# submarine0418/underwater_image_enhancement

Measured on AMD Instinct MI355X. Metric: megapixels/sec enhanced, higher is better.
Workload: dtype f32/f64

## Files before the change

underwater_image_enhancement_amd/csrc/common.h:

```cpp
#pragma once
#include <hip/hip_runtime.h>
#include <stddef.h>
#include <stdint.h>

#include "../../include/uwie.h"

namespace uwie {

void set_error(const char *fmt, ...);
#define UWIE_HIP_CHECK(expr)                                                            \
    do {                                                                                \
        hipError_t _e = (expr);                                                         \
        if (_e != hipSuccess) {                                                         \
            ::uwie::set_error("%s failed: %s (%s:%d)", #expr, hipGetErrorString(_e), __FILE__, __LINE__); \
            return UWIE_E_HIP;                                                          \
        }                                                                               \
    } while (0)
#define UWIE_LAUNCH_CHECK() UWIE_HIP_CHECK(hipGetLastError())
#define UWIE_REQUIRE(cond, msg)                 \
    do {                                        \
        if (!(cond)) {                          \
            ::uwie::set_error("%s", msg);       \
            return UWIE_E_INVALID;              \
        }                                       \
    } while (0)

constexpr int kCastBinadeMin = -2;
constexpr int kCastBinades = 34;

struct LabTables {
    uint16_t gamma[256];
    uint16_t cbrt[3072];
    int32_t fwd[9];
    uint8_t invgamma[4096];
    int32_t ltoyf[512];
    int32_t abtoxz[36864];
    int32_t inv[9];
};

struct CastTables {
    uint32_t R[kCastBinades][256];
    uint8_t tie[kCastBinades][256];
    uint32_t RT[256][kCastBinades];
    uint2 RT2[128][kCastBinades];
    uint8_t tiebin[256];
};

void build_lab_tables(LabTables *t);
void build_cast_tables(CastTables *t);

struct Profiler;
Profiler *prof_create();
void prof_destroy(Profiler *p);
void prof_enable(Profiler *p, bool on);
void prof_filter(Profiler *p, const char *name);
void prof_bind(Profiler *p);
int prof_collect(Profiler *p);
int prof_row(Profiler *p, int i, const char **name, double *ms, int *calls);
class ProfScope {
public:
    ProfScope(const char *name, hipStream_t st);
    ~ProfScope();
    ProfScope(const ProfScope &) = delete;

private:
    int rec_;
    hipStream_t st_;
};
#define UWIE_PROF_CAT2(a, b) a##b
#define UWIE_PROF_CAT(a, b) UWIE_PROF_CAT2(a, b)
#define UWIE_PROF(name, st) ::uwie::ProfScope UWIE_PROF_CAT(_uwie_prof_, __LINE__)(name, st)
#define UWIE_LAUNCH(kernel, grid, block, lds, st, ...)                      \
    do {                                                                    \
        UWIE_PROF(#kernel, st);                                             \
        hipLaunchKernelGGL(kernel, grid, block, lds, st, __VA_ARGS__);      \
    } while (0)

}

namespace uwie {
struct Tuning {
    int gf_pipe = 1;
    int gf_split = 1;
    int gf_bands = 0;
    int select_generic = 0;
    int restore_store = 0;
    int lin_predict3 = 0;
    int lin_cap = 0;
    int lin_no_predict = 0;
    int q_hist = 1;
    int lin_predict_shift = 0;
    int streams = 1;
    int canny_prepass = 1;
    int gf_fuse = 0;
    int rank_sweep = 1;
    int canny_fault_inject = 0;
    int exact_fused = 1;
    int entry_fuse = 1;
};
const Tuning &tune();
uwie_ctx *current_ctx();
}

struct uwie_ctx {
    int device;
    uwie::Tuning tune;
    bool attr_q_tail = false;
    bool attr_cast_resolve = false;
    int attr_gf_fast = 0;
    int attr_gf_split8 = 0;
    uwie::LabTables *d_lab;
    uwie::CastTables *d_cast;
    uwie::Profiler *prof;
    uint32_t *d_status = nullptr;
    hipStream_t aux[4];
    hipEvent_t fork, join[4];
    bool aux_ready;
};

namespace uwie {

struct Carver {
    char *base;
    size_t off;
    explicit Carver(void *b) : base(static_cast<char *>(b)), off(0) {}
    template <typename T>
    T *take(size_t count)
    {
        off = (off + 255) & ~size_t(255);
        T *p = base ? reinterpret_cast<T *>(base + off) : nullptr;
        off += count * sizeof(T);
        return p;
    }
    size_t total() const { return (off + 255) & ~size_t(255); }
};

static inline int cdiv(long long a, long long b) { return (int)((a + b - 1) / b); }
static inline int grid_for(size_t n, size_t cap = 8192)
{
    size_t g = (n + 255) / 256;
    if (g > cap) g = cap;
    return g < 1 ? 1 : (int)g;
}

struct Region {
    int32_t img, y0, x0, rows, cols;
};

struct Shape {
    int B, H, W;
    size_t npx() const { return (size_t)H * W; }
};

size_t cast_ws_bytes(Shape s);
struct EntryFuse {
    uint32_t *qpart;
    uint8_t *gray;
    int32_t *guess;
    int gray_shift;
};
int launch_cast_classify(uwie_ctx *ctx, const uint8_t *d_in, Shape s, int32_t *d_kind, float *d_mean, void *ws,
                         hipStream_t st, const EntryFuse *ef = nullptr);
size_t quad_part_bytes(Shape s);
int launch_quad_hist_reduce(const uint32_t *qpart, Shape s, uint32_t *d_hist, hipStream_t st);
int launch_set_kind(int32_t *d_kind, int B, int kind, hipStream_t st);
int launch_normalise_correct(const uint8_t *d_in, const int32_t *d_kind, float *d_out, Shape s, hipStream_t st);
int launch_quant_gray(const uint8_t *d_in, const int32_t *d_kind, uint8_t *d_gray, Shape s, int gray_shift,
                      hipStream_t st);

size_t airlight_ws_bytes(Shape s);
int launch_airlight(uwie_ctx *ctx, const uint8_t *d_in, const int32_t *d_kind, uint8_t *d_gray, Shape s, int min_size,
                    float *d_A, void *d_trace, void *ws, hipStream_t st, int make_gray_shift = 0, const uint32_t *qpart = nullptr);
bool entry_fuse_takes(Shape s, int min_size);

size_t canny_ws_bytes(Shape s);
int launch_canny(const uint8_t *d_gray, Shape s, const Region *d_regions, int nreg, int max_rows, int max_cols, int low,
                 int high, uint32_t *d_count, uint8_t *d_edges, void *ws, hipStream_t st, bool count_is_zeroed = false,
                 bool strong_is_zeroed = false, bool prepass_done = false);
bool gray_strong_takes(Shape s);
int launch_gray_strong(const uint8_t *d_in, const int32_t *d_kind, uint8_t *d_gray, Shape s, const Region *d_regions, int nreg,
                       int max_rows, int max_cols, int high, int gray_shift, void *ws, hipStream_t st);
int launch_hist_strong(const uint8_t *d_in, const uint8_t *d_gray, Shape s, const Region *d_regions, int nreg, int max_rows,
                       int max_cols, int high, uint32_t *d_hist, void *ws, hipStream_t st);
uint32_t *canny_strong_flags(void *ws, Shape s);
int launch_make_full_regions(Region *d_regions, Shape s, hipStream_t st);

int launch_region_stats(const uint8_t *d_in, const int32_t *d_kind, const Region *d_regs, int nreg, int max_rows,
                        int max_cols, Shape s, float *csum, int maxChunks, float *tot, float *mean, float *vtot,
                        hipStream_t st);
int launch_frame_hist(const uint8_t *d_in, Shape s, uint32_t *d_hist, hipStream_t st);
size_t features_ws_bytes(Shape s);
int launch_features_u8(const uint8_t *d_in, Shape s, float *d_out, void *ws, hipStream_t st);

// ... 165 lines not shown
```

underwater_image_enhancement_amd/csrc/k_guided_pipe.hip:

```cpp
#include "common.h"
#include "devutil.h"
#include "guided_wave.h"

#include <algorithm>
#include <cmath>
#include <type_traits>
#include <utility>

namespace uwie {

namespace {

#define UWIE_TRY_RC(call)               \
    do {                                \
        const int _rc = (call);         \
        if (_rc != UWIE_OK) return _rc; \
    } while (0)

#ifndef UWIE_GF_MINBAND
#define UWIE_GF_MINBAND 32
#endif
constexpr int kPipeSlots = 128;
struct PipeGeom {
    int H, W, band;
// ... 463 lines not shown
        if constexpr (S == 0) {
            const double o0 = x0, o1 = x1;
            x0 = b0; x1 = b1;
            b0 = o0; b1 = o1;
        } else rest.template swap_at<S - 1>(b0, b1);
    }
    __device__ __forceinline__ void clear() { x0 = x1 = 0.0; rest.clear(); }
};
template <>
struct RegRing<0> {
    template <int S> __device__ __forceinline__ void swap_at(double &, double &) {}
    __device__ __forceinline__ void clear() {}
};

template <int N, bool G>
struct RawRing {
    uint32_t t0, t1, g;
    RawRing<N - 1, G> rest;
    template <int S>
    __device__ __forceinline__ void swap_at(uint32_t &a0, uint32_t &a1, uint32_t &gg)
    {
        if constexpr (S == 0) {
            const uint32_t o0 = t0, o1 = t1;
            t0 = a0; t1 = a1;
            a0 = o0; a1 = o1;
            if constexpr (G) {
                const uint32_t og = g;
                g = gg;
                gg = og;
            }
        } else rest.template swap_at<S - 1>(a0, a1, gg);
    }
    template <int S>
    __device__ __forceinline__ void set_at(uint32_t a0, uint32_t a1, uint32_t gg)
    {
        if constexpr (S == 0) {
            t0 = a0; t1 = a1;
            if constexpr (G) g = gg;
        } else rest.template set_at<S - 1>(a0, a1, gg);
    }
};
template <bool G>
struct RawRing<0, G> {
    template <int S> __device__ __forceinline__ void swap_at(uint32_t &, uint32_t &, uint32_t &) {}
    template <int S> __device__ __forceinline__ void set_at(uint32_t, uint32_t, uint32_t) {}
};

#ifndef SPLIT_QUAD
#define SPLIT_QUAD 1
#endif
#ifndef SPLIT_MUL24
#define SPLIT_MUL24 1
#endif
__device__ __forceinline__ double dpp_next(double v)
{
    const int lo = __builtin_amdgcn_update_dpp(0, __double2loint(v), 0x130, 0xf, 0xf, true);
    const int hi = __builtin_amdgcn_update_dpp(0, __double2hiint(v), 0x130, 0xf, 0xf, true);
    return __hiloint2double(hi, lo);
}
__device__ __forceinline__ uint32_t dpp_next(uint32_t v)
{
    return (uint32_t)__builtin_amdgcn_update_dpp(0, (int)v, 0x130, 0xf, 0xf, true);
}
__device__ __forceinline__ double2 q_add(double2 a, double2 b) { return make_double2(a.x + b.x, a.y + b.y); }
__device__ __forceinline__ double2 q_sub(double2 a, double2 b) { return make_double2(a.x - b.x, a.y - b.y); }
__device__ __forceinline__ double2 q_next(double2 v) { return make_double2(dpp_next(v.x), dpp_next(v.y)); }
__device__ __forceinline__ uint2 q_add(uint2 a, uint2 b) { return make_uint2(a.x + b.x, a.y + b.y); }
__device__ __forceinline__ uint2 q_sub(uint2 a, uint2 b) { return make_uint2(a.x - b.x, a.y - b.y); }
__device__ __forceinline__ uint2 q_next(uint2 v) { return make_uint2(dpp_next(v.x), dpp_next(v.y)); }

template <int K>
struct SplitCfg {
    static constexpr bool RAWREG = K <= 16;
    static constexpr int NB = K % 3 == 0 ? 3 : K > 16 ? 2 : K % 5 == 0 ? 5 : 2;
    static constexpr int AR = K > 16 ? 3 : 0;
    static constexpr bool STAGE_FIRST = AR > 0;
    static constexpr int pad_bytes = 16 * (PipeCfg<K>::M + 1) > 128 ? 16 * (PipeCfg<K>::M + 1) : 128;
    static constexpr int s2_bytes = STAGE_FIRST ? 2048 : 2048 + pad_bytes;
    static constexpr int ring_lds_bytes = (K - AR) * (PipeCfg<K>::NL + 1) * 16;
    static_assert(!STAGE_FIRST || ring_lds_bytes >= pad_bytes, "the look-ahead must stay inside the allocation");
    static constexpr int lds_bytes = ring_lds_bytes + PipeCfg<K>::s1_doubles * 8 + s2_bytes;
};

__device__ __forceinline__ uint32_t fuse_t0_bits(const float *tab, uint32_t r, uint32_t g, uint32_t b, float omega, int pre_clip)
{
    const float dark = fminf(fminf(tab[r], tab[256 + g]), tab[512 + b]);
    float t = __fsub_rn(1.0f, __fmul_rn(omega, dark));
    if (pre_clip) t = fminf(fmaxf(t, 0.1f), 1.0f);
    return __float_as_uint(t);
}

template <int K, bool EDGE, typename TOut, bool FUSE = false>
__device__ __forceinline__ void split_body(const uint8_t *__restrict__ gray, const float *__restrict__ t0, TOut *__restrict__ tout,
                                           const SplitGeom &g, const PipeConsts &cs, char *lds, int3 bid, int lane_in = -1,
                                           const float *tab = nullptr, float omega = 0.0f, int pre_clip = 0)
{
    using C = PipeCfg<K>;
    constexpr int a = C::a, Lb = C::Lb, NV = C::NV, RC = K, NL = C::NL, M = C::M, SW = C::SW;
    constexpr int NB = SplitCfg<K>::NB;
    static_assert(RC % NB == 0, "the ring period must be a multiple of the row buffers");
    constexpr bool RAWREG = SplitCfg<K>::RAWREG;
    constexpr int NLp = NL + 1, EB = 16;
    constexpr int AR = SplitCfg<K>::AR;
    constexpr int ring_bytes = SplitCfg<K>::ring_lds_bytes;
    constexpr uint32_t stage_base = SplitCfg<K>::STAGE_FIRST ? 0u : (uint32_t)ring_bytes;
    constexpr uint32_t ring_base = SplitCfg<K>::STAGE_FIRST ? 3072u + 2048u : 0u;
    constexpr double K2 = (double)(K * K);
    const int lane = lane_in >= 0 ? lane_in : (int)threadIdx.x;
    const int H = g.H, W = g.W;
    const int x_lo = bid.x * NV;
    const int y_lo = g.y0 + bid.y * g.band;
    const int r_lo = y_lo - a;
    const size_t img = (size_t)bid.z * H * W;
    const uint32_t npx = (uint32_t)H * (uint32_t)W;
    constexpr uint32_t kTB = FUSE ? 3u : 4u;
    const __amdgpu_buffer_rsrc_t rT = FUSE ? pipe_rsrc(reinterpret_cast<const uint8_t *>(t0) + img * 3, npx * 3u) : pipe_rsrc(t0 + img, npx * 4u),
                                 rG = pipe_rsrc(gray + img, npx), rO = pipe_rsrc(tout + img, npx * (uint32_t)sizeof(TOut));
    const uint32_t pitch_t = (uint32_t)W * kTB, pitch_g = (uint32_t)W, pitch_o = (uint32_t)W * (uint32_t)sizeof(TOut);

    const int xo0 = x_lo + 2 * lane;
    int craw[2], fix_addr[2];
    bool fix_need[2], fix_odd[2];
    uint32_t ofs_t[2], ofs_g[2], ofs_o[2], ofs_q[2];
#pragma unroll
    for (int j = 0; j < 2; ++j) {
        const int sl = 2 * lane + j;
        craw[j] = EDGE ? pipe_reflect(x_lo - 2 * a + sl, W) : x_lo - 2 * a + sl;
        ofs_t[j] = (uint32_t)craw[j] * kTB;
        ofs_g[j] = (uint32_t)craw[j];
        ofs_o[j] = EDGE ? (uint32_t)min(xo0 + j, W - 1) : (uint32_t)min(xo0, W - 2);
        ofs_q[j] = sl < NV && xo0 + j < W ? (uint32_t)(xo0 + j) * (uint32_t)sizeof(TOut) : kNoStore;
        const int c = x_lo - a + sl, cr = pipe_reflect(c, W);
        const int sp = min(max(cr - (x_lo - a), 0), kPipeSlots - 1);
        fix_need[j] = EDGE && cr != c;
        fix_addr[j] = (sp >> 1) << 2;
        fix_odd[j] = sp & 1;
    }

    const uint32_t a_ring = pipe_opaque(ring_base + (uint32_t)min(lane, NLp - 1) * (uint32_t)EB);

#ifndef SPLIT_RAW_G
#define SPLIT_RAW_G 1
#endif
    constexpr bool RAWG = SPLIT_RAW_G && RAWREG && K == 15 && !FUSE;
    struct In {
        uint32_t te[2];
        uint32_t ge[2], go[2];
        uint32_t gl[2];
        uint32_t tl[2];
    };
    auto byte_of = [](const uint32_t (&v)[2], int c) { return EDGE ? v[c] : (c == 0 ? (v[0] & 255u) : (v[0] >> 8)); };
    static_assert(!FUSE || RAWREG, "the fused transmission keeps its rows in the register ring (no leaving-row reload)");
    auto load_rows = [&](uint32_t oe_t, uint32_t oe_g, uint32_t ol_t, uint32_t ol_g, uint32_t oo_g, In &in) {
        if constexpr (!RAWREG) {
            if constexpr (!EDGE) {
                const u32x2 tl = __builtin_amdgcn_raw_buffer_load_b64(rT, ofs_t[0], ol_t, 0);
                in.tl[0] = tl.x; in.tl[1] = tl.y;
            } else {
                in.tl[0] = (uint32_t)__builtin_amdgcn_raw_buffer_load_b32(rT, ofs_t[0], ol_t, 0);
                in.tl[1] = (uint32_t)__builtin_amdgcn_raw_buffer_load_b32(rT, ofs_t[1], ol_t, 0);
            }
        }
        if constexpr (!RAWG) {
            if constexpr (!EDGE) in.gl[0] = (uint16_t)__builtin_amdgcn_raw_buffer_load_b16(rG, ofs_g[0], ol_g, 0);
            else {
                in.gl[0] = (uint8_t)__builtin_amdgcn_raw_buffer_load_b8(rG, ofs_g[0], ol_g, 0);
                in.gl[1] = (uint8_t)__builtin_amdgcn_raw_buffer_load_b8(rG, ofs_g[1], ol_g, 0);
            }
        }
        if constexpr (!EDGE) {
            if constexpr (FUSE) {
                in.te[0] = (uint32_t)__builtin_amdgcn_raw_buffer_load_b32(rT, ofs_t[0], oe_t, 0);
                in.te[1] = (uint16_t)__builtin_amdgcn_raw_buffer_load_b16(rT, ofs_t[0] + 4u, oe_t, 0);
            } else {
                const u32x2 te = __builtin_amdgcn_raw_buffer_load_b64(rT, ofs_t[0], oe_t, 0);
                in.te[0] = te.x; in.te[1] = te.y;
            }
            in.ge[0] = (uint16_t)__builtin_amdgcn_raw_buffer_load_b16(rG, ofs_g[0], oe_g, 0);
            in.go[0] = (uint16_t)__builtin_amdgcn_raw_buffer_load_b16(rG, ofs_o[0], oo_g, 0);
            in.ge[1] = in.go[1] = 0;
        } else {
#pragma unroll
            for (int j = 0; j < 2; ++j) {
                if constexpr (FUSE) {
                    const uint32_t r = (uint8_t)__builtin_amdgcn_raw_buffer_load_b8(rT, ofs_t[j], oe_t, 0);
                    const uint32_t gg = (uint8_t)__builtin_amdgcn_raw_buffer_load_b8(rT, ofs_t[j] + 1u, oe_t, 0);
                    const uint32_t bb = (uint8_t)__builtin_amdgcn_raw_buffer_load_b8(rT, ofs_t[j] + 2u, oe_t, 0);
                    in.te[j] = r | (gg << 8) | (bb << 16);
                } else {
                    in.te[j] = (uint32_t)__builtin_amdgcn_raw_buffer_load_b32(rT, ofs_t[j], oe_t, 0);
                }
                in.ge[j] = (uint8_t)__builtin_amdgcn_raw_buffer_load_b8(rG, ofs_g[j], oe_g, 0);
                in.go[j] = (uint8_t)__builtin_amdgcn_raw_buffer_load_b8(rG, ofs_o[j], oo_g, 0);
            }
        }
    };
    auto te_bits = [&](const In &in, uint32_t (&tb)[2]) {
        if constexpr (!FUSE) {
            tb[0] = in.te[0]; tb[1] = in.te[1];
        } else if constexpr (!EDGE) {
            const uint32_t w0 = in.te[0], w1 = in.te[1];
            tb[0] = fuse_t0_bits(tab, w0 & 255u, (w0 >> 8) & 255u, (w0 >> 16) & 255u, omega, pre_clip);
            tb[1] = fuse_t0_bits(tab, w0 >> 24, w1 & 255u, (w1 >> 8) & 255u, omega, pre_clip);
        } else {
#pragma unroll
            for (int j = 0; j < 2; ++j)
                tb[j] = fuse_t0_bits(tab, in.te[j] & 255u, (in.te[j] >> 8) & 255u, (in.te[j] >> 16) & 255u, omega, pre_clip);
        }
    };

    double V1p[2] = {0.0, 0.0}, V1gp[2] = {0.0, 0.0};
    uint32_t Sg[2] = {0, 0}, Sgg[2] = {0, 0};
    double V2a[2] = {0.0, 0.0}, V2b[2] = {0.0, 0.0};
    RawRing<RAWREG ? RC : 0, RAWG> raw;
    auto prologue_row = [&](auto j_tag) {
        constexpr int J = decltype(j_tag)::value;
        const uint32_t row = (uint32_t)pipe_reflect(r_lo - a + J, H);
        uint32_t tb[2], gq[2];
#pragma unroll
        for (int c = 0; c < 2; ++c) {
            gq[c] = (uint8_t)__builtin_amdgcn_raw_buffer_load_b8(rG, ofs_g[c], row * pitch_g, 0);
            if constexpr (FUSE) {
                const uint32_t r = (uint8_t)__builtin_amdgcn_raw_buffer_load_b8(rT, ofs_t[c], row * pitch_t, 0);
                const uint32_t gg = (uint8_t)__builtin_amdgcn_raw_buffer_load_b8(rT, ofs_t[c] + 1u, row * pitch_t, 0);
                const uint32_t bb = (uint8_t)__builtin_amdgcn_raw_buffer_load_b8(rT, ofs_t[c] + 2u, row * pitch_t, 0);
                tb[c] = fuse_t0_bits(tab, r, gg, bb, omega, pre_clip);
            } else {
                tb[c] = (uint32_t)__builtin_amdgcn_raw_buffer_load_b32(rT, ofs_t[c], row * pitch_t, 0);
            }
            const double p = (double)__uint_as_float(tb[c]);
            Sg[c] += gq[c];
            Sgg[c] += gq[c] * gq[c];
            V1p[c] += p;
            V1gp[c] += (double)gq[c] * p;
        }
        if constexpr (RAWREG) raw.template set_at<J>(tb[0], tb[1], gq[0] | (gq[1] << 8));
    };
    [&]<int... J>(std::integer_sequence<int, J...>) { (prologue_row(IC<J>{}), ...); }(std::make_integer_sequence<int, RC>{});
    RegRing<RC> rb;
    rb.clear();
#pragma unroll
    for (int s = 0; s < RC - AR; ++s) *reinterpret_cast<double2 *>(lds + a_ring + (uint32_t)(s * NLp * EB)) = make_double2(0.0, 0.0);
    RegRing<AR> ra;
    ra.clear();

    const uint32_t a16 = pipe_opaque(stage_base + (uint32_t)lane * 16u);
    const uint32_t a8 = pipe_opaque(stage_base + 2048u + (uint32_t)lane * 8u);
    const double2 *pp1 = reinterpret_cast<const double2 *>(lds + a16), *vv1 = pp1 + SW;
    const uint2 *pi = reinterpret_cast<const uint2 *>(lds + a8), *vi = pi + SW;
    const double2 *pp2 = reinterpret_cast<const double2 *>(lds + a16 + 3072u), *vv2 = pp2 + SW;
    static_assert(C::s1_doubles * 8 == 3072 && (SplitCfg<K>::STAGE_FIRST || SplitCfg<K>::s2_bytes >= 2048 + 16 * (C::M + 1)), "staging layout");
    auto window2 = [&](const double2 *pp, const double2 *vv, double2 P, double2 v1, double2 (&o)[2]) {
        double2 m0 = pp[1], m1 = pp[2];
#pragma unroll
        for (int d = 3; d < M; d += 2) { const double2 t = pp[d]; m0.x += t.x; m0.y += t.y; }
#pragma unroll
        for (int d = 4; d < M; d += 2) { const double2 t = pp[d]; m1.x += t.x; m1.y += t.y; }
        const double2 f0 = vv[M];
        const double midx = m0.x + m1.x, midy = m0.y + m1.y;
        if constexpr (K & 1) {
            const double2 pm = pp[M];
            o[0] = make_double2((P.x + midx) + f0.x, (P.y + midy) + f0.y);
            o[1] = make_double2((v1.x + midx) + pm.x, (v1.y + midy) + pm.y);
        } else {
            o[0] = make_double2(P.x + midx, P.y + midy);
            o[1] = make_double2((v1.x + midx) + f0.x, (v1.y + midy) + f0.y);
        }
    };
    constexpr bool QUAD = SPLIT_QUAD != 0 && ((K & 1) || !(M & 1));
    static_assert(!QUAD || !(K & 1) || (M & 1), "odd windows: an odd number of pair sums on either side of the lane's own");
    double2 keep1 = make_double2(0.0, 0.0), keep2 = keep1;
    uint2 keepI = make_uint2(0u, 0u);
    auto stage_q = [&](auto *line, auto s0, auto s1, auto &keep) {
        const auto P = q_add(s0, s1);
        const auto Pn = q_next(P);
        const auto R = q_add(P, Pn);
        line[0] = R;
        if constexpr (K & 1) {
            line[SW] = s1;
            keep = q_add(s1, Pn);
        } else {
            line[SW] = s0;
            keep = R;
        }
    };
    auto window_q = [&](const auto *rr, auto keep, auto s0, auto s1, auto *o) {
        using T = decltype(keep);
        const T w = rr[SW + M];
        if constexpr (K & 1) {
            T mid = rr[2];
#pragma unroll
            for (int d = 4; d <= M - 3; d += 2) mid = q_add(mid, rr[d]);
            o[1] = q_add(q_add(keep, mid), rr[M - 1]);
            o[0] = q_add(q_sub(o[1], w), s0);
        } else if constexpr (!(M & 1)) {
            T mid = rr[2];
#pragma unroll
            for (int d = 4; d <= M - 2; d += 2) mid = q_add(mid, rr[d]);
            o[0] = q_add(keep, mid);
            o[1] = q_add(q_sub(o[0], s0), w);
        } else {
            T mid = rr[1];
#pragma unroll
            for (int d = 3; d <= M - 2; d += 2) mid = q_add(mid, rr[d]);
            o[0] = q_add(q_add(s0, s1), mid);
            o[1] = q_add(q_add(s1, mid), w);
        }
    };
    auto stage_v1 = [&]() {
        if constexpr (QUAD) {
            stage_q(const_cast<double2 *>(pp1), make_double2(V1p[0], V1gp[0]), make_double2(V1p[1], V1gp[1]), keep1);
            stage_q(const_cast<uint2 *>(pi), make_uint2(Sg[0], Sgg[0]), make_uint2(Sg[1], Sgg[1]), keepI);
        } else {
            const_cast<double2 *>(pp1)[0] = make_double2(V1p[0] + V1p[1], V1gp[0] + V1gp[1]);
            const_cast<double2 *>(vv1)[0] = make_double2(V1p[0], V1gp[0]);
            const_cast<uint2 *>(pi)[0] = make_uint2(Sg[0] + Sg[1], Sgg[0] + Sgg[1]);
            const_cast<uint2 *>(vi)[0] = make_uint2(Sg[0], Sgg[0]);
        }
    };

    auto step = [&](auto warm_tag, auto slot_tag, const In &in, uint32_t orow, bool row_ok) {
        constexpr bool WARM = decltype(warm_tag)::value;
        constexpr int S = decltype(slot_tag)::value;
        char *ring_p = lds + a_ring + (uint32_t)((S >= AR ? S - AR : 0) * NLp * EB);
        double2 oab[2] = {make_double2(0.0, 0.0), make_double2(0.0, 0.0)};
        if constexpr (!WARM) {
            if constexpr (QUAD) window_q(pp2, keep2, make_double2(V2a[0], V2b[0]), make_double2(V2a[1], V2b[1]), oab);
            else window2(pp2, vv2, make_double2(V2a[0] + V2a[1], V2b[0] + V2b[1]), make_double2(V2a[1], V2b[1]), oab);
        }
        double2 opg[2];
        if constexpr (QUAD) window_q(pp1, keep1, make_double2(V1p[0], V1gp[0]), make_double2(V1p[1], V1gp[1]), opg);
        else window2(pp1, vv1, make_double2(V1p[0] + V1p[1], V1gp[0] + V1gp[1]), make_double2(V1p[1], V1gp[1]), opg);
        uint32_t oG[2], oGG[2];
        if constexpr (QUAD) {
            uint2 oi[2];
            window_q(pi, keepI, make_uint2(Sg[0], Sgg[0]), make_uint2(Sg[1], Sgg[1]), oi);
            oG[0] = oi[0].x; oGG[0] = oi[0].y;
            oG[1] = oi[1].x; oGG[1] = oi[1].y;
        } else {
            const uint2 *ps = pi;
            uint2 m0 = ps[1], m1 = ps[2];
#pragma unroll
            for (int d = 3; d < M; d += 2) { m0.x += ps[d].x; m0.y += ps[d].y; }
#pragma unroll
            for (int d = 4; d < M; d += 2) { m1.x += ps[d].x; m1.y += ps[d].y; }
            const uint32_t midg = m0.x + m1.x, midgg = m0.y + m1.y;
            const uint2 f0 = vi[M];
            if constexpr (K & 1) {
                const uint2 pm = ps[M];
                oG[0] = Sg[0] + Sg[1] + midg + f0.x;   oGG[0] = Sgg[0] + Sgg[1] + midgg + f0.y;
                oG[1] = Sg[1] + midg + pm.x;           oGG[1] = Sgg[1] + midgg + pm.y;
            } else {
                oG[0] = Sg[0] + Sg[1] + midg;          oGG[0] = Sgg[0] + Sgg[1] + midgg;
                oG[1] = Sg[1] + midg + f0.x;           oGG[1] = Sgg[1] + midgg + f0.y;
            }
        }
        double2 la = make_double2(0.0, 0.0);
        if constexpr (S >= AR) la = *reinterpret_cast<const double2 *>(ring_p);

        if constexpr (!WARM) {
#pragma unroll
            for (int c = 0; c < 2; ++c) {
                const double gd = (double)byte_of(in.go, c);
                const double q = fmin(fmax(fma(oab[c].x * cs.kaI, gd, fma(oab[c].y, cs.kb, cs.b0)), 0.1), 1.0);
                const uint32_t oq = row_ok ? ofs_q[c] : kNoStore;
                if constexpr (std::is_same<TOut, double>::value)
                    __builtin_amdgcn_raw_buffer_store_b64(__builtin_bit_cast(u32x2, q), rO, oq, orow, 0);
                else
                    __builtin_amdgcn_raw_buffer_store_b32(__float_as_uint((float)q), rO, oq, orow, 0);
            }
        }
        double av[2], bv[2];
#pragma unroll
        for (int c = 0; c < 2; ++c) {
            constexpr bool MUL24 = SPLIT_MUL24 && 255 * 255 * K * K < (1 << 24);
            const uint32_t nvar = MUL24 ? __umul24(oGG[c], (uint32_t)(K * K)) - __umul24(oG[c], oG[c])
                                        : oGG[c] * (uint32_t)(K * K) - oG[c] * oG[c];
            const double D = fma((double)nvar, 1.0 / 255.0, cs.Ek);
            const double gd = (double)oG[c];
            const double ncov = fma(K2, opg[c].y, -(gd * opg[c].x));
            av[c] = ncov * pipe_rcp(D);
            bv[c] = fma(av[c] * (-1.0 / 255.0), gd, opg[c].x) * (1.0 / K2);
        }
        if constexpr (EDGE) {
            double fa[2] = {av[0], av[1]}, fb[2] = {bv[0], bv[1]};
#pragma unroll
            for (int c = 0; c < 2; ++c) {
                auto bp = [&](double v) {
                    const int lo = __builtin_amdgcn_ds_bpermute(fix_addr[c], __double2loint(v));
                    const int hi = __builtin_amdgcn_ds_bpermute(fix_addr[c], __double2hiint(v));
                    return __hiloint2double(hi, lo);
                };
                const double a0 = bp(av[0]), a1 = bp(av[1]), b0 = bp(bv[0]), b1 = bp(bv[1]);
                if (fix_need[c]) {
                    fa[c] = fix_odd[c] ? a1 : a0;
                    fb[c] = fix_odd[c] ? b1 : b0;
                }
            }
            av[0] = fa[0]; av[1] = fa[1];
            bv[0] = fb[0]; bv[1] = fb[1];
        }
        double lb0 = bv[0], lb1 = bv[1];
        rb.template swap_at<S>(lb0, lb1);
        if constexpr (S < AR) {
            la = make_double2(av[0], av[1]);
            ra.template swap_at<S>(la.x, la.y);
        }
        V2a[0] += av[0] - la.x; V2a[1] += av[1] - la.y;
        V2b[0] += bv[0] - lb0;  V2b[1] += bv[1] - lb1;
        uint32_t tbe[2];
        te_bits(in, tbe);
        uint32_t lt[2] = {tbe[0], tbe[1]}, lg = EDGE ? (in.ge[0] | (in.ge[1] << 8)) : in.ge[0];
        if constexpr (RAWREG) raw.template swap_at<S>(lt[0], lt[1], lg);
        else { lt[0] = in.tl[0]; lt[1] = in.tl[1]; }
        if constexpr (!RAWG) lg = EDGE ? (in.gl[0] | (in.gl[1] << 8)) : in.gl[0];
#pragma unroll
        for (int c = 0; c < 2; ++c) {
            const double pe = (double)__uint_as_float(tbe[c]), pl = (double)__uint_as_float(lt[c]);
            const uint32_t ge = byte_of(in.ge, c), gl = c == 0 ? (lg & 255u) : (lg >> 8);
            Sg[c] += ge - gl;
            Sgg[c] += ge * ge - gl * gl;
            V1p[c] += pe - pl;
            V1gp[c] += (double)ge * pe - (double)gl * pl;
        }

        pipe_sync();
        stage_v1();
        if constexpr (QUAD) {
            stage_q(const_cast<double2 *>(pp2), make_double2(V2a[0], V2b[0]), make_double2(V2a[1], V2b[1]), keep2);
        } else {
            const_cast<double2 *>(pp2)[0] = make_double2(V2a[0] + V2a[1], V2b[0] + V2b[1]);
            const_cast<double2 *>(vv2)[0] = make_double2(V2a[0], V2b[0]);
        }
        if constexpr (S >= AR) *reinterpret_cast<double2 *>(ring_p) = make_double2(av[0], av[1]);
        pipe_sync();
    };

    pipe_sync();
    stage_v1();
    pipe_sync();
    const int i0 = r_lo + 1;
    int re = i0 + Lb;
    int gr = i0 - Lb - 2;
    int yo = y_lo;
    auto issue = [&](In &fill) {
        asm volatile("" : "+s"(re), "+s"(gr), "+s"(yo));
        const uint32_t er = (uint32_t)pipe_reflect(re, H), lr = (uint32_t)pipe_reflect(re - RC, H);
        const uint32_t og = (uint32_t)min(max(gr, 0), H - 1);
        load_rows(er * pitch_t, er * pitch_g, lr * pitch_t, lr * pitch_g, og * pitch_g, fill);
        ++re;
        ++gr;
    };
    In buf[NB];
    [&]<int... Q>(std::integer_sequence<int, Q...>) { (issue(buf[Q]), ...); }(std::make_integer_sequence<int, NB - 1>{});
    auto one = [&](auto warm_tag, auto slot_tag, In &fill, const In &use) {
        issue(fill);
        step(warm_tag, slot_tag, use, (uint32_t)yo * pitch_o, yo < H);
        if constexpr (!decltype(warm_tag)::value) ++yo;
        __builtin_amdgcn_sched_barrier(0);
    };
    auto period = [&](auto warm_tag) {
        auto at = [&](auto slot_tag) {
            constexpr int S = decltype(slot_tag)::value;
            one(warm_tag, slot_tag, buf[(S + NB - 1) % NB], buf[S % NB]);
        };
        [&]<int... Q>(std::integer_sequence<int, Q...>) { (at(IC<Q>{}), ...); }(std::make_integer_sequence<int, RC>{});
    };
    period(std::true_type{});
    const int nper = (((int)bid.y == g.nbands - 1 ? g.y_end - y_lo : g.band) + RC - 1) / RC;
    for (int p = 0; p < nper; ++p) period(std::false_type{});
}


template <int K, typename TOut>
__global__ void __launch_bounds__(64) __attribute__((amdgpu_waves_per_eu(2, 2)))
k_guided_split(const uint8_t *__restrict__ gray, const float *__restrict__ t0, TOut *__restrict__ tout, SplitGeom g, PipeConsts cs)
{
    extern __shared__ double2 lds_raw[];
    char *lds = reinterpret_cast<char *>(lds_raw);
    int3 bid = {(int)blockIdx.x, (int)blockIdx.y, (int)blockIdx.z};
    if (g.xcd_fold) {
        const uint32_t gx = gridDim.x, gy = gridDim.y, n = gx * gy * gridDim.z;
        const uint32_t lin = blockIdx.x + gx * (blockIdx.y + gy * blockIdx.z);
        const uint32_t xcd = lin & 7u, idx = lin >> 3, q = n >> 3, r = n & 7u;
        const uint32_t log = (xcd < r ? xcd * (q + 1) : r * (q + 1) + (xcd - r) * q) + idx;
        bid.x = (int)(log % gx);
        bid.y = (int)((log / gx) % gy);
        bid.z = (int)(log / (gx * gy));
    }
    const int x_lo = bid.x * PipeCfg<K>::NV;
    const bool edge = x_lo - 2 * PipeCfg<K>::a < 0 || x_lo - 2 * PipeCfg<K>::a + kPipeSlots > g.W;
    if (edge) split_body<K, true, TOut>(gray, t0, tout, g, cs, lds, bid);
    else split_body<K, false, TOut>(gray, t0, tout, g, cs, lds, bid);
}

struct FuseT0Args {
    const uint8_t *rgb;
    const int32_t *kind;
    const float *A;
    float omega, norm_eps;
    int pre_clip;
};

template <int K, typename TOut>
__global__ void __launch_bounds__(512) __attribute__((amdgpu_waves_per_eu(2, 2)))
k_guided_split8(const uint8_t *__restrict__ gray, FuseT0Args fz, TOut *__restrict__ tout, SplitGeom g, PipeConsts cs, int nstrips)
{
    extern __shared__ double2 lds_raw[];
    char *lds = reinterpret_cast<char *>(lds_raw);
    constexpr int per_wave = SplitCfg<K>::lds_bytes;
    float *tab = reinterpret_cast<float *>(lds + 8 * per_wave);
    const int wave = __builtin_amdgcn_readfirstlane((int)(threadIdx.x >> 6)), lane = threadIdx.x & 63;
    int grp = (int)blockIdx.x, b = (int)blockIdx.z;
    if (g.xcd_fold) {
        const uint32_t gx = gridDim.x, n = gx * gridDim.z, lin = blockIdx.x + gx * blockIdx.z;
        const uint32_t xcd = lin & 7u, idx = lin >> 3, q = n >> 3, r = n & 7u;
        const uint32_t log = (xcd < r ? xcd * (q + 1) : r * (q + 1) + (xcd - r) * q) + idx;
        grp = (int)(log % gx);
        b = (int)(log / gx);
    }
    {
        const int kd = fz.kind ? fz.kind[b] : 0;
        for (int i = threadIdx.x; i < 768; i += 512) {
            const int c = i >> 8;
            tab[i] = px_val(i & 255, px_atten(kd, c)) / (fz.A[b * 3 + c] + fz.norm_eps);
        }
    }
    __syncthreads();
    const int item = grp * 8 + wave;
    if (item >= nstrips * g.nbands) return;
    const int3 bid = {item % nstrips, item / nstrips, b};
    const int x_lo = bid.x * PipeCfg<K>::NV;
    const bool edge = x_lo - 2 * PipeCfg<K>::a < 0 || x_lo - 2 * PipeCfg<K>::a + kPipeSlots > g.W;
    const float *t0 = reinterpret_cast<const float *>(fz.rgb);
    if (edge) split_body<K, true, TOut, true>(gray, t0, tout, g, cs, lds + wave * per_wave, bid, lane, tab, fz.omega, fz.pre_clip);
    else split_body<K, false, TOut, true>(gray, t0, tout, g, cs, lds + wave * per_wave, bid, lane, tab, fz.omega, fz.pre_clip);
}

template <int K, typename TOut>
int launch_split8(const uint8_t *d_gray, const FuseT0Args &fz, Shape s, const PipeConsts &cs, TOut *d_t, int y0, int band, int nbands,
                  int y_end, hipStream_t st)
{
    using C = PipeCfg<K>;
    constexpr int lds = 8 * SplitCfg<K>::lds_bytes + 768 * 4;
    static_assert(lds <= 160 * 1024, "eight strips and the table have to fit one CU");
#ifndef UWIE_SPLIT8_FOLD
#define UWIE_SPLIT8_FOLD 1
#endif
    SplitGeom g{s.H, s.W, y0, band, y_end, UWIE_SPLIT8_FOLD, nbands};
    const int nstrips = cdiv(s.W, C::NV);
    uwie_ctx *ctx = current_ctx();
    const int bit = std::is_same<TOut, double>::value ? 1 : 2;
    if (ctx && !(ctx->attr_gf_split8 & bit)) {
        UWIE_HIP_CHECK(hipFuncSetAttribute(reinterpret_cast<const void *>(&k_guided_split8<K, TOut>),
                                           hipFuncAttributeMaxDynamicSharedMemorySize, lds));
        ctx->attr_gf_split8 |= bit;
    }
    {
        UWIE_PROF("k_guided_split8", st);
        hipLaunchKernelGGL((k_guided_split8<K, TOut>), dim3(cdiv((long long)nstrips * nbands, 8), 1, s.B), dim3(512), (size_t)lds, st, d_gray,
                           fz, d_t, g, cs, nstrips);
    }
    UWIE_LAUNCH_CHECK();
    return UWIE_OK;
}

template <int K, typename TOut>
int launch_split(const uint8_t *d_gray, const float *d_t0, Shape s, const PipeConsts &cs, TOut *d_t, int y0, int band, int nbands,
                 int y_end, hipStream_t st)
{
    using C = PipeCfg<K>;
    constexpr int lds = SplitCfg<K>::lds_bytes;
#ifndef UWIE_SPLIT_FOLD
#define UWIE_SPLIT_FOLD 1
#endif
    SplitGeom g{s.H, s.W, y0, band, y_end, UWIE_SPLIT_FOLD, nbands};
    const int nstrips = cdiv(s.W, C::NV);
    {
        UWIE_PROF("k_guided_split", st);
        hipLaunchKernelGGL((k_guided_split<K, TOut>), dim3(nstrips, nbands, s.B), dim3(64), (size_t)lds, st, d_gray, d_t0, d_t, g, cs);
    }
    UWIE_LAUNCH_CHECK();
    return UWIE_OK;
}

template <int K, bool FX, typename TOut>
int launch_pipe(const uint8_t *d_gray, const float *d_t0, Shape s, const PipeConsts &cs, TOut *d_t, hipStream_t st,
                const int *border = nullptr)
{
    using C = PipeCfg<K>;
    constexpr int lds = C::lds_bytes(FX);
    const int nstrips = cdiv(s.W, C::NV);
    const int resident = 256 * std::max(1, std::min(8, (160 * 1024) / lds));
    int nbands = 1;
    if (tune().gf_bands > 0) nbands = tune().gf_bands;
    else {
        const long strips = (long)nstrips * s.B;
        if (strips < 12L * resident) nbands = (int)cdiv((size_t)(12L * resident), (size_t)strips);
        const int cap = std::max(1, s.H / (16 * (K - 1)));
        nbands = std::min(nbands, std::max(cap, (int)cdiv((size_t)(3L * resident), (size_t)strips)));
    }
    nbands = std::max(1, std::min(nbands, s.H / std::max(UWIE_GF_MINBAND, 2 * K)));
    PipeGeom g{};
    g.H = s.H; g.W = s.W;
    g.band = cdiv(s.H, nbands);
    int gy = cdiv(s.H, g.band);
    if (border) {
        g.iy0 = border[0]; g.iy1 = border[1]; g.iband = border[2];
        gy = 2 + border[3];
        g.is0 = border[4]; g.is1 = border[5];
    }
    {
        UWIE_PROF("k_guided_pipe", st);
        hipLaunchKernelGGL((k_guided_pipe<K, FX, TOut>), dim3(nstrips, gy, s.B), dim3(64), (size_t)lds, st, d_gray, d_t0, d_t, g, cs);
    }
    UWIE_LAUNCH_CHECK();
    return UWIE_OK;
}

}

bool guided_split_plan(Shape s, int k, int *iy0, int *band, int *nb, int *rows)
{
    if (rows) *rows = 0;
    if ((k != 10 && k != 15 && k != 20) || (s.W & 1) || !tune().gf_split) return false;
    if (s.W < 2 * k || s.H < 4 * k || s.B > 65535 || s.npx() >= ((size_t)1 << 27)) return false;
    const int RC = k, a = k / 2, Lb = k - 1 - a, NV = kPipeSlots - 2 * (k - 1);
    const bool odd = k & 1;
    *iy0 = odd ? 0 : 2 * a;
    const int periods = odd ? cdiv(s.H, RC) : (s.H - 2 * a - 2 * Lb) / RC;
    if (periods < 4) return false;
    const long strips = (long)cdiv(s.W, NV) * s.B;
    const bool forced = tune().gf_bands > 0;
    int n;
    if (forced) n = tune().gf_bands;
    else {
        n = (int)cdiv((size_t)(8L * 2048), (size_t)strips);
        n = std::min(n, std::max(1, periods * RC / 180));
    }
    n = std::max(1, std::min(n, periods));
    if (odd) {
        const int per_band = cdiv(periods, n);
        *band = RC * per_band;
        *nb = cdiv(periods, per_band);
        if (rows) *rows = s.H;
    } else {
        const int per_band = periods / n;
        *band = RC * per_band;
        *nb = periods / per_band;
        if (rows) *rows = periods * RC;
    }
    return forced || strips * n >= 1024;
}

bool guided_fused_takes(Shape s, int k)
{
    if (k != 15 || !tune().gf_pipe || !tune().gf_fuse) return false;
    int iy0, band, nb, rows;
// ... 114 lines not shown
```

Measured before the change: 57010.

## Compute fused dark-channel transmission in registers and enable guided-filter fusion by default

The fused guided-filter split kernel now computes the initial transmission from RGB directly in registers, using per-image reciprocal divisors (StretchDiv) and packed float2 math. This replaces the per-block LDS lookup table that was built by 512-thread blocks. The kernel goes back to 64-thread single-strip blocks that use the normal split LDS footprint, and it computes the next row's transmission one step ahead to hide ALU latency. gf_fuse is switched on by default, so the fused path that skips a separate t0 pass now runs. In exchange there is more per-pixel arithmetic and register pressure, and a slower exact-division variant is used when the fast divisor is not valid.

Measured after the change: 59170, median of 6. 1.04x the previous value.

```diff
diff --git a/underwater_image_enhancement_amd/csrc/common.h b/underwater_image_enhancement_amd/csrc/common.h
--- a/underwater_image_enhancement_amd/csrc/common.h
+++ b/underwater_image_enhancement_amd/csrc/common.h
@@ -92,7 +92,7 @@
     int lin_predict_shift = 0;
     int streams = 1;
     int canny_prepass = 1;
-    int gf_fuse = 0;
+    int gf_fuse = 1;
     int rank_sweep = 1;
     int canny_fault_inject = 0;
     int exact_fused = 1;
@@ -108,7 +108,6 @@
     bool attr_q_tail = false;
     bool attr_cast_resolve = false;
     int attr_gf_fast = 0;
-    int attr_gf_split8 = 0;
     uwie::LabTables *d_lab;
     uwie::CastTables *d_cast;
     uwie::Profiler *prof;
diff --git a/underwater_image_enhancement_amd/csrc/k_guided_pipe.hip b/underwater_image_enhancement_amd/csrc/k_guided_pipe.hip
--- a/underwater_image_enhancement_amd/csrc/k_guided_pipe.hip
+++ b/underwater_image_enhancement_amd/csrc/k_guided_pipe.hip
@@ -569,18 +569,72 @@
     static constexpr int lds_bytes = ring_lds_bytes + PipeCfg<K>::s1_doubles * 8 + s2_bytes;
 };
 
-__device__ __forceinline__ uint32_t fuse_t0_bits(const float *tab, uint32_t r, uint32_t g, uint32_t b, float omega, int pre_clip)
-{
-    const float dark = fminf(fminf(tab[r], tab[256 + g]), tab[512 + b]);
-    float t = __fsub_rn(1.0f, __fmul_rn(omega, dark));
-    if (pre_clip) t = fminf(fmaxf(t, 0.1f), 1.0f);
-    return __float_as_uint(t);
-}
-
-template <int K, bool EDGE, typename TOut, bool FUSE = false>
+struct FuseT0Args {
+    const uint8_t *rgb;
+    const int32_t *kind;
+    const float *A;
+    float omega, norm_eps;
+    int pre_clip;
+};
+struct T0Regs {
+    StretchDiv dv[3];
+    float att1, att2;
+    float omega;
+    int pre_clip;
+    __device__ __forceinline__ bool set(const FuseT0Args &fz, int b)
+    {
+        auto uni = [](float v) { return __int_as_float(__builtin_amdgcn_readfirstlane(__float_as_int(v))); };
+        const int kd = fz.kind ? fz.kind[b] : 0;
+        bool fast = true;
+#pragma unroll
+        for (int c = 0; c < 3; ++c) {
+            dv[c].set(fz.A[b * 3 + c] + fz.norm_eps);
+            dv[c].den = uni(dv[c].den);
+            dv[c].y = uni(dv[c].y);
+            fast = fast && dv[c].fast;
+        }
+        att1 = uni(px_atten(kd, 1) ? 0.85f : 1.0f);
+        att2 = uni(px_atten(kd, 2) ? 0.85f : 1.0f);
+        omega = uni(fz.omega);
+        pre_clip = fz.pre_clip;
+        return fast;
+    }
+};
+typedef float f32x2 __attribute__((ext_vector_type(2)));
+template <int FUSE>
+__device__ __forceinline__ void reg_t0_bits2(const T0Regs &z, const uint32_t (&px)[2], uint32_t (&tb)[2])
+{
+    auto chan = [&](auto c_tag) {
+        constexpr int c = decltype(c_tag)::value;
+        const f32x2 x = {(float)((px[0] >> (8 * c)) & 255u), (float)((px[1] >> (8 * c)) & 255u)};
+        const float rcp = 1.0f / 255.0f;
+        const f32x2 q0 = x * rcp;
+        f32x2 n = __builtin_elementwise_fma(__builtin_elementwise_fma(-q0, f32x2{255.0f, 255.0f}, x), f32x2{rcp, rcp}, q0);
+        if constexpr (c == 1) n = n * z.att1;
+        if constexpr (c == 2) n = n * z.att2;
+        const StretchDiv &d = z.dv[c];
+        if constexpr (FUSE == 1) {
+            const f32x2 nd = {-d.den, -d.den}, yy = {d.y, d.y};
+            f32x2 q = n * d.y;
+            q = __builtin_elementwise_fma(__builtin_elementwise_fma(nd, q, n), yy, q);
+            return __builtin_elementwise_fma(__builtin_elementwise_fma(nd, q, n), yy, q);
+        } else {
+            return f32x2{n.x / d.den, n.y / d.den};
+        }
+    };
+    const f32x2 q0 = chan(IC<0>{}), q1 = chan(IC<1>{}), q2 = chan(IC<2>{});
+    const float dark[2] = {fminf(fminf(q0.x, q1.x), q2.x), fminf(fminf(q0.y, q1.y), q2.y)};
+#pragma unroll
+    for (int j = 0; j < 2; ++j) {
+        float t = __fsub_rn(1.0f, __fmul_rn(z.omega, dark[j]));
+        if (z.pre_clip) t = fminf(fmaxf(t, 0.1f), 1.0f);
+        tb[j] = __float_as_uint(t);
+    }
+}
+
+template <int K, bool EDGE, typename TOut, int FUSE = 0>
 __device__ __forceinline__ void split_body(const uint8_t *__restrict__ gray, const float *__restrict__ t0, TOut *__restrict__ tout,
-                                           const SplitGeom &g, const PipeConsts &cs, char *lds, int3 bid, int lane_in = -1,
-                                           const float *tab = nullptr, float omega = 0.0f, int pre_clip = 0)
+                                           const SplitGeom &g, const PipeConsts &cs, char *lds, int3 bid, const T0Regs *z = nullptr)
 {
     using C = PipeCfg<K>;
     constexpr int a = C::a, Lb = C::Lb, NV = C::NV, RC = K, NL = C::NL, M = C::M, SW = C::SW;
@@ -593,7 +647,7 @@
     constexpr uint32_t stage_base = SplitCfg<K>::STAGE_FIRST ? 0u : (uint32_t)ring_bytes;
     constexpr uint32_t ring_base = SplitCfg<K>::STAGE_FIRST ? 3072u + 2048u : 0u;
     constexpr double K2 = (double)(K * K);
-    const int lane = lane_in >= 0 ? lane_in : (int)threadIdx.x;
+    const int lane = (int)threadIdx.x;
     const int H = g.H, W = g.W;
     const int x_lo = bid.x * NV;
     const int y_lo = g.y0 + bid.y * g.band;
@@ -687,12 +741,9 @@
             tb[0] = in.te[0]; tb[1] = in.te[1];
         } else if constexpr (!EDGE) {
             const uint32_t w0 = in.te[0], w1 = in.te[1];
-            tb[0] = fuse_t0_bits(tab, w0 & 255u, (w0 >> 8) & 255u, (w0 >> 16) & 255u, omega, pre_clip);
-            tb[1] = fuse_t0_bits(tab, w0 >> 24, w1 & 255u, (w1 >> 8) & 255u, omega, pre_clip);
-        } else {
-#pragma unroll
-            for (int j = 0; j < 2; ++j)
-                tb[j] = fuse_t0_bits(tab, in.te[j] & 255u, (in.te[j] >> 8) & 255u, (in.te[j] >> 16) & 255u, omega, pre_clip);
+            reg_t0_bits2<FUSE>(*z, {w0 & 0xffffffu, (w0 >> 24) | ((w1 & 0xffffu) << 8)}, tb);
+        } else {
+            reg_t0_bits2<FUSE>(*z, in.te, tb);
         }
     };
 
@@ -711,10 +762,17 @@
                 const uint32_t r = (uint8_t)__builtin_amdgcn_raw_buffer_load_b8(rT, ofs_t[c], row * pitch_t, 0);
                 const uint32_t gg = (uint8_t)__builtin_amdgcn_raw_buffer_load_b8(rT, ofs_t[c] + 1u, row * pitch_t, 0);
                 const uint32_t bb = (uint8_t)__builtin_amdgcn_raw_buffer_load_b8(rT, ofs_t[c] + 2u, row * pitch_t, 0);
-                tb[c] = fuse_t0_bits(tab, r, gg, bb, omega, pre_clip);
+                tb[c] = r | (gg << 8) | (bb << 16);
             } else {
                 tb[c] = (uint32_t)__builtin_amdgcn_raw_buffer_load_b32(rT, ofs_t[c], row * pitch_t, 0);
             }
+        }
+        if constexpr (FUSE) {
+            const uint32_t px[2] = {tb[0], tb[1]};
+            reg_t0_bits2<FUSE>(*z, px, tb);
+        }
+#pragma unroll
+        for (int c = 0; c < 2; ++c) {
             const double p = (double)__uint_as_float(tb[c]);
             Sg[c] += gq[c];
             Sgg[c] += gq[c] * gq[c];
@@ -806,7 +864,9 @@
         }
     };
 
-    auto step = [&](auto warm_tag, auto slot_tag, const In &in, uint32_t orow, bool row_ok) {
+    uint32_t tnext[2] = {0u, 0u};
+    static_assert(!FUSE || NB >= 3, "the next step's row has to be loaded a step ahead of the refill");
+    auto step = [&](auto warm_tag, auto slot_tag, const In &in, const In &nxt, uint32_t orow, bool row_ok) {
         constexpr bool WARM = decltype(warm_tag)::value;
         constexpr int S = decltype(slot_tag)::value;
         char *ring_p = lds + a_ring + (uint32_t)((S >= AR ? S - AR : 0) * NLp * EB);
@@ -896,7 +956,8 @@
         V2a[0] += av[0] - la.x; V2a[1] += av[1] - la.y;
         V2b[0] += bv[0] - lb0;  V2b[1] += bv[1] - lb1;
         uint32_t tbe[2];
-        te_bits(in, tbe);
+        if constexpr (FUSE != 0) { tbe[0] = tnext[0]; tbe[1] = tnext[1]; }
+        else te_bits(in, tbe);
         uint32_t lt[2] = {tbe[0], tbe[1]}, lg = EDGE ? (in.ge[0] | (in.ge[1] << 8)) : in.ge[0];
         if constexpr (RAWREG) raw.template swap_at<S>(lt[0], lt[1], lg);
         else { lt[0] = in.tl[0]; lt[1] = in.tl[1]; }
@@ -920,6 +981,7 @@
             const_cast<double2 *>(vv2)[0] = make_double2(V2a[0], V2b[0]);
         }
         if constexpr (S >= AR) *reinterpret_cast<double2 *>(ring_p) = make_double2(av[0], av[1]);
+        if constexpr (FUSE != 0) te_bits(nxt, tnext);
         pipe_sync();
     };
 
@@ -940,16 +1002,17 @@
     };
     In buf[NB];
     [&]<int... Q>(std::integer_sequence<int, Q...>) { (issue(buf[Q]), ...); }(std::make_integer_sequence<int, NB - 1>{});
-    auto one = [&](auto warm_tag, auto slot_tag, In &fill, const In &use) {
+    if constexpr (FUSE != 0) te_bits(buf[0], tnext);
+    auto one = [&](auto warm_tag, auto slot_tag, In &fill, const In &use, const In &nxt) {
         issue(fill);
-        step(warm_tag, slot_tag, use, (uint32_t)yo * pitch_o, yo < H);
+        step(warm_tag, slot_tag, use, nxt, (uint32_t)yo * pitch_o, yo < H);
         if constexpr (!decltype(warm_tag)::value) ++yo;
         __builtin_amdgcn_sched_barrier(0);
     };
     auto period = [&](auto warm_tag) {
         auto at = [&](auto slot_tag) {
             constexpr int S = decltype(slot_tag)::value;
-            one(warm_tag, slot_tag, buf[(S + NB - 1) % NB], buf[S % NB]);
+            one(warm_tag, slot_tag, buf[(S + NB - 1) % NB], buf[S % NB], buf[(S + 1) % NB]);
         };
         [&]<int... Q>(std::integer_sequence<int, Q...>) { (at(IC<Q>{}), ...); }(std::make_integer_sequence<int, RC>{});
     };
@@ -959,12 +1022,11 @@
 }
 
 
-template <int K, typename TOut>
-__global__ void __launch_bounds__(64) __attribute__((amdgpu_waves_per_eu(2, 2)))
-k_guided_split(const uint8_t *__restrict__ gray, const float *__restrict__ t0, TOut *__restrict__ tout, SplitGeom g, PipeConsts cs)
-{
-    extern __shared__ double2 lds_raw[];
-    char *lds = reinterpret_cast<char *>(lds_raw);
+#ifndef UWIE_SPLIT_FOLD
+#define UWIE_SPLIT_FOLD 1
+#endif
+__device__ __forceinline__ int3 split_bid(const SplitGeom &g)
+{
     int3 bid = {(int)blockIdx.x, (int)blockIdx.y, (int)blockIdx.z};
     if (g.xcd_fold) {
         const uint32_t gx = gridDim.x, gy = gridDim.y, n = gx * gy * gridDim.z;
@@ -975,53 +1037,41 @@
         bid.y = (int)((log / gx) % gy);
         bid.z = (int)(log / (gx * gy));
     }
+    return bid;
+}
+
+template <int K, typename TOut>
+__global__ void __launch_bounds__(64) __attribute__((amdgpu_waves_per_eu(2, 2)))
+k_guided_split(const uint8_t *__restrict__ gray, const float *__restrict__ t0, TOut *__restrict__ tout, SplitGeom g, PipeConsts cs)
+{
+    extern __shared__ double2 lds_raw[];
+    char *lds = reinterpret_cast<char *>(lds_raw);
+    const int3 bid = split_bid(g);
     const int x_lo = bid.x * PipeCfg<K>::NV;
     const bool edge = x_lo - 2 * PipeCfg<K>::a < 0 || x_lo - 2 * PipeCfg<K>::a + kPipeSlots > g.W;
     if (edge) split_body<K, true, TOut>(gray, t0, tout, g, cs, lds, bid);
     else split_body<K, false, TOut>(gray, t0, tout, g, cs, lds, bid);
 }
 
-struct FuseT0Args {
-    const uint8_t *rgb;
-    const int32_t *kind;
-    const float *A;
-    float omega, norm_eps;
-    int pre_clip;
-};
-
 template <int K, typename TOut>
-__global__ void __launch_bounds__(512) __attribute__((amdgpu_waves_per_eu(2, 2)))
-k_guided_split8(const uint8_t *__restrict__ gray, FuseT0Args fz, TOut *__restrict__ tout, SplitGeom g, PipeConsts cs, int nstrips)
+__global__ void __launch_bounds__(64) __attribute__((amdgpu_waves_per_eu(2, 2)))
+k_guided_split8(const uint8_t *__restrict__ gray, FuseT0Args fz, TOut *__restrict__ tout, SplitGeom g, PipeConsts cs)
 {
     extern __shared__ double2 lds_raw[];
     char *lds = reinterpret_cast<char *>(lds_raw);
-    constexpr int per_wave = SplitCfg<K>::lds_bytes;
-    float *tab = reinterpret_cast<float *>(lds + 8 * per_wave);
-    const int wave = __builtin_amdgcn_readfirstlane((int)(threadIdx.x >> 6)), lane = threadIdx.x & 63;
-    int grp = (int)blockIdx.x, b = (int)blockIdx.z;
-    if (g.xcd_fold) {
-        const uint32_t gx = gridDim.x, n = gx * gridDim.z, lin = blockIdx.x + gx * blockIdx.z;
-        const uint32_t xcd = lin & 7u, idx = lin >> 3, q = n >> 3, r = n & 7u;
-        const uint32_t log = (xcd < r ? xcd * (q + 1) : r * (q + 1) + (xcd - r) * q) + idx;
-        grp = (int)(log % gx);
-        b = (int)(log / gx);
-    }
-    {
-        const int kd = fz.kind ? fz.kind[b] : 0;
-        for (int i = threadIdx.x; i < 768; i += 512) {
-            const int c = i >> 8;
-            tab[i] = px_val(i & 255, px_atten(kd, c)) / (fz.A[b * 3 + c] + fz.norm_eps);
-        }
-    }
-    __syncthreads();
-    const int item = grp * 8 + wave;
-    if (item >= nstrips * g.nbands) return;
-    const int3 bid = {item % nstrips, item / nstrips, b};
+    const int3 bid = split_bid(g);
     const int x_lo = bid.x * PipeCfg<K>::NV;
     const bool edge = x_lo - 2 * PipeCfg<K>::a < 0 || x_lo - 2 * PipeCfg<K>::a + kPipeSlots > g.W;
+    T0Regs z;
+    const bool fast = z.set(fz, bid.z);
     const float *t0 = reinterpret_cast<const float *>(fz.rgb);
-    if (edge) split_body<K, true, TOut, true>(gray, t0, tout, g, cs, lds + wave * per_wave, bid, lane, tab, fz.omega, fz.pre_clip);
-    else split_body<K, false, TOut, true>(gray, t0, tout, g, cs, lds + wave * per_wave, bid, lane, tab, fz.omega, fz.pre_clip);
+    if (fast) {
+        if (edge) split_body<K, true, TOut, 1>(gray, t0, tout, g, cs, lds, bid, &z);
+        else split_body<K, false, TOut, 1>(gray, t0, tout, g, cs, lds, bid, &z);
+    } else {
+        if (edge) split_body<K, true, TOut, 2>(gray, t0, tout, g, cs, lds, bid, &z);
+        else split_body<K, false, TOut, 2>(gray, t0, tout, g, cs, lds, bid, &z);
+    }
 }
 
 template <int K, typename TOut>
@@ -1029,24 +1079,12 @@
                   int y_end, hipStream_t st)
 {
     using C = PipeCfg<K>;
-    constexpr int lds = 8 * SplitCfg<K>::lds_bytes + 768 * 4;
-    static_assert(lds <= 160 * 1024, "eight strips and the table have to fit one CU");
-#ifndef UWIE_SPLIT8_FOLD
-#define UWIE_SPLIT8_FOLD 1
-#endif
-    SplitGeom g{s.H, s.W, y0, band, y_end, UWIE_SPLIT8_FOLD, nbands};
+    constexpr int lds = SplitCfg<K>::lds_bytes;
+    SplitGeom g{s.H, s.W, y0, band, y_end, UWIE_SPLIT_FOLD, nbands};
     const int nstrips = cdiv(s.W, C::NV);
-    uwie_ctx *ctx = current_ctx();
-    const int bit = std::is_same<TOut, double>::value ? 1 : 2;
-    if (ctx && !(ctx->attr_gf_split8 & bit)) {
-        UWIE_HIP_CHECK(hipFuncSetAttribute(reinterpret_cast<const void *>(&k_guided_split8<K, TOut>),
-                                           hipFuncAttributeMaxDynamicSharedMemorySize, lds));
-        ctx->attr_gf_split8 |= bit;
-    }
     {
         UWIE_PROF("k_guided_split8", st);
-        hipLaunchKernelGGL((k_guided_split8<K, TOut>), dim3(cdiv((long long)nstrips * nbands, 8), 1, s.B), dim3(512), (size_t)lds, st, d_gray,
-                           fz, d_t, g, cs, nstrips);
+        hipLaunchKernelGGL((k_guided_split8<K, TOut>), dim3(nstrips, nbands, s.B), dim3(64), (size_t)lds, st, d_gray, fz, d_t, g, cs);
     }
     UWIE_LAUNCH_CHECK();
     return UWIE_OK;
@@ -1058,9 +1096,6 @@
 {
     using C = PipeCfg<K>;
     constexpr int lds = SplitCfg<K>::lds_bytes;
-#ifndef UWIE_SPLIT_FOLD
-#define UWIE_SPLIT_FOLD 1
-#endif
     SplitGeom g{s.H, s.W, y0, band, y_end, UWIE_SPLIT_FOLD, nbands};
     const int nstrips = cdiv(s.W, C::NV);
     {
```
